# google-research/big_vision

Hardware: NVIDIA H100
Metric: siglip_vit_b16_pairs_per_sec (higher is better)
Workload: dtype bf16

## Files before the change

### big_vision_b200/csrc/gemm.cu

```cuda
#include "common.cuh"
#include "gemm_sched.h"
#include "host_utils.h"
#include "kernels.h"

#include <atomic>

#include <stdlib.h>
#include <string.h>

namespace bv {

namespace {

constexpr int BM = 128;
constexpr int BK = 64;
constexpr int A_STAGE_BYTES = BM * BK * 2;
constexpr int NUM_THREADS = 384;
constexpr int SUB_BYTES = 64 * 64 * 2;

enum : int { EF_BIAS = 0, EF_GELU = 1, EF_RESID = 2, EF_DGELU = 3 };
enum : int { OM_F32 = 0, OM_BF16_ADD = 1, OM_BF16_TMA = 2 };

template <int BN, int OM, int EF>
struct Cfg {
  static constexpr int B_STAGE_BYTES = BN * BK * 2;
  static constexpr int STAGE_BYTES = A_STAGE_BYTES + B_STAGE_BYTES;
  static constexpr int OUTS = OM != OM_BF16_TMA ? 0 : (EF == EF_GELU ? 2 : 1);
  static constexpr int BUF_BYTES = OUTS * SUB_BYTES;
  static constexpr int STAGING_BYTES = 2 * 2 * BUF_BYTES;
  static constexpr int SMEM_LIMIT = 232448 - 2048;
  static constexpr int STAGES_FIT = (SMEM_LIMIT - STAGING_BYTES) / STAGE_BYTES;
  static constexpr int STAGES = STAGES_FIT > 8 ? 8 : STAGES_FIT;
  static constexpr int STAGING_OFFSET = STAGES * STAGE_BYTES;
  static constexpr int BAR_OFFSET = STAGING_OFFSET + STAGING_BYTES;
  static constexpr int SMEM_BYTES = BAR_OFFSET + 256 + 1024;
  static_assert(STAGES >= 3, "shared-memory budget leaves fewer than 3 stages");
};

struct GemmDev {
  GemmSched s;
  int M, N;
  int a_mn, b_mn;
  int reduce_out;
  float alpha;
  const float* bias;
  const bf16* aux;
  void* d; void* d2;
  long long ldd, ldd2, ldaux;
  float* colsum;
  int aux_row_mod;
};

template <int BN, int STAGES, int STAGE_BYTES, int TA, int TB>
__device__ __forceinline__ void mainloop(float (&acc)[BN / 2], uint32_t base, uint32_t bar_base, int cw,
                                         PipeState& ps, int kb0, int kb1) {
  constexpr uint32_t a_lbo = TA ? 8192u : 16u, b_lbo = TB ? 8192u : 16u;
  constexpr uint32_t a_kstep = TA ? 2048u : 32u, b_kstep = TB ? 2048u : 32u;
  int prev_stage = -1;
  for (int kb = kb0; kb < kb1; ++kb) {
    mbar_wait(bar_base + 8u * ps.stage, ps.phase);
    const uint32_t a_s = base + ps.stage * STAGE_BYTES + cw * 8192;
    const uint32_t b_s = base + ps.stage * STAGE_BYTES + A_STAGE_BYTES;
    const uint64_t adesc = wgmma_desc_sw128(a_s, a_lbo, 1024u), bdesc = wgmma_desc_sw128(b_s, b_lbo, 1024u);
    wgmma_fence_regs(acc);
    wgmma_fence();
#pragma unroll
    for (int k = 0; k < BK / 16; ++k) {
      const uint64_t a = adesc + k * (a_kstep >> 4), b = bdesc + k * (b_kstep >> 4);
      const int accumulate = (kb > kb0 || k > 0) ? 1 : 0;
      if constexpr (BN == 256) wgmma_ss_n256<TA, TB>(acc, a, b, accumulate);
      else wgmma_ss_n128<TA, TB>(acc, a, b, accumulate);
    }
    wgmma_commit();
    wgmma_fence_regs(acc);
    wgmma_wait<1>();
    if (prev_stage >= 0 && (threadIdx.x & 127) == 0) mbar_arrive(bar_base + 8u * (STAGES + prev_stage));
    prev_stage = ps.stage;
    ps.advance(STAGES);
  }
  wgmma_wait<0>();
  wgmma_fence_regs(acc);
  if (prev_stage >= 0 && (threadIdx.x & 127) == 0) mbar_arrive(bar_base + 8u * (STAGES + prev_stage));
}

template <bool OUT_F32, int EF>
__device__ __forceinline__ void epi_math(const GemmDev& p, float alpha, float c0, float c1, float b0, float b1,
                                         int row, int col, bool pair, float& v0, float& v1, float& pre0,
                                         float& pre1) {
  constexpr bool HAS_AUX = (EF == EF_RESID || EF == EF_DGELU);
  v0 = c0 * alpha + b0;
  v1 = c1 * alpha + b1;
  float a0 = 0.f, a1 = 0.f;
  if (HAS_AUX) {
    const long long ar = p.aux_row_mod > 0 ? (row % p.aux_row_mod) : row;
    const bf16* ap = p.aux + ar * p.ldaux + col;
    if (pair) {
      const uint32_t q = *reinterpret_cast<const uint32_t*>(ap);
      a0 = bf16_lo(q); a1 = bf16_hi(q);
    } else {
      a0 = __bfloat162float(*ap);
    }
  }
  pre0 = pre1 = 0.f;
  if (EF == EF_GELU) {
    pre0 = round_bf16(v0); pre1 = round_bf16(v1);
    v0 = gelu_tanh_fast(pre0); v1 = gelu_tanh_fast(pre1);
  } else if (EF == EF_RESID) {
    v0 = (OUT_F32 ? v0 : round_bf16(v0)) + a0;
    v1 = (OUT_F32 ? v1 : round_bf16(v1)) + a1;
  } else if (EF == EF_DGELU) {
    v0 *= gelu_tanh_grad_fast(a0);
    v1 *= gelu_tanh_grad_fast(a1);
  }
}


__device__ __forceinline__ void colsum_add(float* colsum, int N, float s0, float s1, int col, int lane) {
  s0 += __shfl_xor_sync(0xffffffffu, s0, 4);
  s0 += __shfl_xor_sync(0xffffffffu, s0, 8);
  s0 += __shfl_xor_sync(0xffffffffu, s0, 16);
  s1 += __shfl_xor_sync(0xffffffffu, s1, 4);
  s1 += __shfl_xor_sync(0xffffffffu, s1, 8);
  s1 += __shfl_xor_sync(0xffffffffu, s1, 16);
  if (lane < 4) {
    if (col < N) atomicAdd(colsum + col, s0);
    if (col + 1 < N) atomicAdd(colsum + col + 1, s1);
  }
}

template <int BN, bool OUT_F32, int EF>
__device__ __forceinline__ void epilogue_regs(const GemmDev& p, const float (&acc)[BN / 2], int m0, int n0,
                                              int cw) {
  const int lane = threadIdx.x & 31, warp = (threadIdx.x >> 5) & 3;
  const int row0 = m0 + cw * 64 + warp * 16 + (lane >> 2);
  const int pM = p.M, pN = p.N;
  const float alpha = p.alpha;
  const bool reduce = p.reduce_out != 0;
#pragma unroll
  for (int j = 0; j < BN / 8; ++j) {
    const int col = n0 + 8 * j + 2 * (lane & 3);
    if (col >= pN) continue;
    const bool pair = col + 1 < pN;
    float b0 = 0.f, b1 = 0.f;
    if (p.bias != nullptr) {
      b0 = __ldg(p.bias + col);
      if (pair) b1 = __ldg(p.bias + col + 1);
    }
#pragma unroll
    for (int h = 0; h < 2; ++h) {
      const int row = row0 + 8 * h;
      if (row >= pM) continue;
      float v0, v1, pre0, pre1;
      epi_math<OUT_F32, EF>(p, alpha, acc[4 * j + 2 * h], acc[4 * j + 2 * h + 1], b0, b1, row, col, pair, v0, v1,
                            pre0, pre1);
      if (OUT_F32) {
        float* dp = static_cast<float*>(p.d) + row * p.ldd + col;
        if (reduce) {
          atomicAdd(dp, v0);
          if (pair) atomicAdd(dp + 1, v1);
        } else if (pair) {
          *reinterpret_cast<float2*>(dp) = make_float2(v0, v1);
        } else {
          *dp = v0;
        }
      } else {
        bf16* dp = static_cast<bf16*>(p.d) + row * p.ldd + col;
        const __nv_bfloat162 o = __floats2bfloat162_rn(v0, v1);
        if (pair) atomicAdd(reinterpret_cast<__nv_bfloat162*>(dp), o);
        else atomicAdd(dp, o.x);
      }
    }
  }
}

template <int BN, int EF, int BUF_BYTES>
__device__ __forceinline__ void epilogue_tma(const GemmDev& p, const CUtensorMap* tmD, const CUtensorMap* tmD2,
                                             const float (&acc)[BN / 2], int m0, int n0, int cw, uint32_t staging,
                                             uint32_t& nstore) {
  const int lane = threadIdx.x & 31, warp = (threadIdx.x >> 5) & 3;
  const bool leader = (threadIdx.x & 127) == 0;
  const int rl0 = warp * 16 + (lane >> 2);
  const int row0 = m0 + cw * 64 + rl0;
  const int pM = p.M, pN = p.N;
  const float alpha = p.alpha;
#pragma unroll
  for (int c = 0; c < BN / 64; ++c) {
    const uint32_t buf = staging + (nstore & 1u) * BUF_BYTES;
    if (leader) tma_store_wait_read<1>();
    named_bar_sync(1 + cw, 128);
    float cs[8][2];
#pragma unroll
    for (int jj = 0; jj < 8; ++jj) {
      const int j = 8 * c + jj;
      const int col = n0 + 8 * j + 2 * (lane & 3);
      cs[jj][0] = cs[jj][1] = 0.f;
      const bool cin = col < pN, pair = col + 1 < pN;
      float b0 = 0.f, b1 = 0.f;
      if (cin && p.bias != nullptr) {
        b0 = __ldg(p.bias + col);
        if (pair) b1 = __ldg(p.bias + col + 1);
      }
#pragma unroll
      for (int h = 0; h < 2; ++h) {
        const int rl = rl0 + 8 * h, row = row0 + 8 * h;
        float v0 = 0.f, v1 = 0.f, pre0 = 0.f, pre1 = 0.f;
        const bool in = cin && row < pM;
        if (in)
          epi_math<false, EF>(p, alpha, acc[4 * j + 2 * h], acc[4 * j + 2 * h + 1], b0, b1, row, col, pair, v0, v1,
                              pre0, pre1);
        const __nv_bfloat162 o = __floats2bfloat162_rn(v0, v1);
        if (in) {
          cs[jj][0] += __low2float(o);
          cs[jj][1] += pair ? __high2float(o) : 0.f;
        }
        const uint32_t off = rl * 128 + ((jj ^ (rl & 7)) << 4) + (lane & 3) * 4;
        asm volatile("st.shared.b32 [%0], %1;" ::"r"(buf + off), "r"(*reinterpret_cast<const uint32_t*>(&o))
                     : "memory");
        if (EF == EF_GELU) {
          const __nv_bfloat162 q = __floats2bfloat162_rn(pre0, pre1);
          asm volatile("st.shared.b32 [%0], %1;" ::"r"(buf + SUB_BYTES + off),
                       "r"(*reinterpret_cast<const uint32_t*>(&q))
                       : "memory");
        }
      }
    }
    fence_proxy_async();
    named_bar_sync(1 + cw, 128);
    if (leader) {
      if (n0 + 64 * c < pN && m0 + cw * 64 < pM) {
        tma_store_2d(tmD, buf, n0 + 64 * c, m0 + cw * 64);
        if (EF == EF_GELU) tma_store_2d(tmD2, buf + SUB_BYTES, n0 + 64 * c, m0 + cw * 64);
      }
      tma_store_commit();
    }
    ++nstore;
    if (p.colsum != nullptr) {
#pragma unroll
      for (int jj = 0; jj < 8; ++jj)
        colsum_add(p.colsum, pN, cs[jj][0], cs[jj][1], n0 + 8 * (8 * c + jj) + 2 * (lane & 3), lane);
    }
  }
}

template <int BN, int OM, int EF>
__global__ void __launch_bounds__(NUM_THREADS, 1)
gemm_kernel(const __grid_constant__ CUtensorMap tmA, const __grid_constant__ CUtensorMap tmB,
            const __grid_constant__ CUtensorMap tmD, const __grid_constant__ CUtensorMap tmD2, const GemmDev p) {
  using C = Cfg<BN, OM, EF>;
  extern __shared__ uint8_t smem_raw[];
  const uint32_t raw_addr = smem_u32(smem_raw);
  const uint32_t base = (raw_addr + 1023u) & ~1023u;
  const uint32_t bar_base = base + C::BAR_OFFSET;
  auto full_bar = [&](int s) { return bar_base + 8u * s; };
  auto empty_bar = [&](int s) { return bar_base + 8u * (C::STAGES + s); };

  const int wg = __shfl_sync(0xffffffffu, static_cast<int>(threadIdx.x >> 7), 0);
  const int units = p.s.units;

  if (threadIdx.x == 0) {
    tma_prefetch_desc(&tmA);
    tma_prefetch_desc(&tmB);
    for (int s = 0; s < C::STAGES; ++s) {
      mbar_init(full_bar(s), 1);
      mbar_init(empty_bar(s), 2);
    }
    fence_barrier_init();
  }
  __syncthreads();

  if (wg == 0) {
    asm volatile("setmaxnreg.dec.sync.aligned.u32 40;");
    if (threadIdx.x == 0) {
      PipeState ps;
      for (int u = blockIdx.x; u < units; u += gridDim.x) {
        const WorkUnit w = gemm_work_unit(p.s, u, BM, BN);
        for (int kb = w.kb0; kb < w.kb1; ++kb) {
          mbar_wait(empty_bar(ps.stage), ps.phase ^ 1u);
          const uint32_t a_s = base + ps.stage * C::STAGE_BYTES;
          const uint32_t b_s = a_s + A_STAGE_BYTES;
          const uint32_t fb = full_bar(ps.stage);
          mbar_expect_tx(fb, C::STAGE_BYTES);
          const int k0 = kb * BK;
          if (p.a_mn) {
#pragma unroll
            for (int j = 0; j < BM / 64; ++j) tma_load_2d(a_s + j * 8192, &tmA, fb, w.m0 + 64 * j, k0);
          } else {
            tma_load_2d(a_s, &tmA, fb, k0, w.m0);
          }
          if (p.b_mn) {
#pragma unroll
            for (int j = 0; j < BN / 64; ++j) tma_load_2d(b_s + j * 8192, &tmB, fb, w.n0 + 64 * j, k0);
          } else {
            tma_load_2d(b_s, &tmB, fb, k0, w.n0);
          }
          ps.advance(C::STAGES);
        }
      }
    }
    return;
  }

  asm volatile("setmaxnreg.inc.sync.aligned.u32 232;");
  const int cw = wg - 1;
  const uint32_t staging = base + C::STAGING_OFFSET + cw * 2 * C::BUF_BYTES;
  uint32_t nstore = 0;
  PipeState ps;
  constexpr int S = C::STAGES, SB = C::STAGE_BYTES;
  for (int u = blockIdx.x; u < units; u += gridDim.x) {
    const WorkUnit w = gemm_work_unit(p.s, u, BM, BN);
    float acc[BN / 2];
    if (p.a_mn) {
      if (p.b_mn) mainloop<BN, S, SB, 1, 1>(acc, base, bar_base, cw, ps, w.kb0, w.kb1);
      else mainloop<BN, S, SB, 1, 0>(acc, base, bar_base, cw, ps, w.kb0, w.kb1);
    } else {
      if (p.b_mn) mainloop<BN, S, SB, 0, 1>(acc, base, bar_base, cw, ps, w.kb0, w.kb1);
      else mainloop<BN, S, SB, 0, 0>(acc, base, bar_base, cw, ps, w.kb0, w.kb1);
    }

    if constexpr (OM == OM_BF16_TMA) epilogue_tma<BN, EF, C::BUF_BYTES>(p, &tmD, &tmD2, acc, w.m0, w.n0, cw, staging, nstore);
    else epilogue_regs<BN, OM == OM_F32, EF>(p, acc, w.m0, w.n0, cw);
  }
  if (OM == OM_BF16_TMA && (threadIdx.x & 127) == 0) tma_store_wait<0>();
}

template <int BN, int OM, int EF>
int launch_cfg(const GemmArgs& g, cudaStream_t stream) {
  using C = Cfg<BN, OM, EF>;
  CUtensorMap tmA, tmB, tmD, tmD2;
  int rc;
  const CUtensorMapDataType bf = CU_TENSOR_MAP_DATA_TYPE_BFLOAT16;
  if (g.a_mn) rc = make_tmap_2d(&tmA, bf, g.A, g.M, g.K, g.lda * 2, 64, 64);
  else        rc = make_tmap_2d(&tmA, bf, g.A, g.K, g.M, g.lda * 2, 64, BM);
  if (rc) return rc;
  if (g.b_mn) rc = make_tmap_2d(&tmB, bf, g.B, g.N, g.K, g.ldb * 2, 64, 64);
  else        rc = make_tmap_2d(&tmB, bf, g.B, g.K, g.N, g.ldb * 2, 64, BN);
  if (rc) return rc;

  GemmDev p;
  const long long tiles = ((g.M + BM - 1) / BM) * ((g.N + BN - 1) / BN);
  if (tiles * ((g.K + BK - 1) / BK) > 0x7fffffffLL) { set_error("bv_gemm: problem too large"); return BV_ERR_INVALID; }
  if (!gemm_make_sched(g.M, g.N, g.K, BM, BN, BK, g.splits, g.reduce_out != 0, num_sms(), &p.s)) {
    set_error("bv_gemm: split-K requires reduce_out=1");
    return BV_ERR_INVALID;
  }
  p.M = (int)g.M; p.N = (int)g.N;
  p.a_mn = g.a_mn; p.b_mn = g.b_mn; p.reduce_out = g.reduce_out;
  p.alpha = g.alpha;
  p.bias = g.bias;
  p.colsum = g.colsum;
  p.aux = reinterpret_cast<const bf16*>(g.aux);
  p.ldaux = g.ldaux;
  p.aux_row_mod = g.aux_row_mod;
  p.d = g.D; p.d2 = g.D2;
  p.ldd = g.ldd; p.ldd2 = g.ldd2;
  memset(&tmD, 0, sizeof(tmD));
  memset(&tmD2, 0, sizeof(tmD2));
  if (OM == OM_BF16_TMA) {
    rc = make_tmap_2d(&tmD, bf, g.D, g.N, g.M, g.ldd * 2, 64, 64);
    if (rc) return rc;
    if (EF == EF_GELU) {
      rc = make_tmap_2d(&tmD2, bf, g.D2, g.N, g.M, g.ldd2 * 2, 64, 64);
      if (rc) return rc;
    }
  }

  auto kern = gemm_kernel<BN, OM, EF>;
  static std::atomic<bool> attr_set[64];
  int dev = 0;
  if (cudaGetDevice(&dev) != cudaSuccess || dev < 0 || dev >= 64) dev = -1;
  if (dev < 0 || !attr_set[dev].load(std::memory_order_acquire)) {
    rc = check_cuda(cudaFuncSetAttribute(kern, cudaFuncAttributeMaxDynamicSharedMemorySize, C::SMEM_BYTES),
                    "cudaFuncSetAttribute(gemm)");
    if (rc) return rc;
    if (dev >= 0) attr_set[dev].store(true, std::memory_order_release);
  }
  const int grid = p.s.units < num_sms() ? p.s.units : num_sms();
  kern<<<grid, NUM_THREADS, C::SMEM_BYTES, stream>>>(tmA, tmB, tmD, tmD2, p);
  return check_cuda(cudaGetLastError(), "gemm_kernel launch");
}

template <int BN>
int dispatch_epi(const GemmArgs& g, cudaStream_t s) {
  const bool f32 = (g.out_dtype == DT_F32), add = !f32 && g.reduce_out;
  switch (g.epi) {
    case EPI_NONE:
    case EPI_BIAS:
      return f32 ? launch_cfg<BN, OM_F32, EF_BIAS>(g, s)
                 : add ? launch_cfg<128, OM_BF16_ADD, EF_BIAS>(g, s) : launch_cfg<BN, OM_BF16_TMA, EF_BIAS>(g, s);
    case EPI_BIAS_RESID:
      return f32 ? launch_cfg<BN, OM_F32, EF_RESID>(g, s)
                 : add ? launch_cfg<128, OM_BF16_ADD, EF_RESID>(g, s) : launch_cfg<BN, OM_BF16_TMA, EF_RESID>(g, s);
    case EPI_BIAS_GELU:
      return launch_cfg<BN, OM_BF16_TMA, EF_GELU>(g, s);
    case EPI_DGELU:
      if (f32) { set_error("bv_gemm: DGELU epilogue writes bf16"); return BV_ERR_INVALID; }
      if (g.aux_row_mod > 0) { set_error("bv_gemm: DGELU takes a row-aligned aux"); return BV_ERR_INVALID; }
      return add ? launch_cfg<128, OM_BF16_ADD, EF_DGELU>(g, s) : launch_cfg<BN, OM_BF16_TMA, EF_DGELU>(g, s);
  }
  set_error("bv_gemm: bad epilogue %d", g.epi);
  return BV_ERR_INVALID;
}

}

int launch_gemm(const GemmArgs& g, cudaStream_t stream) {
  if (g.M <= 0 || g.N <= 0 || g.K <= 0) { set_error("bv_gemm: empty problem"); return BV_ERR_INVALID; }
  if (g.out_dtype == DT_BF16 && ((reinterpret_cast<uintptr_t>(g.D) & 15) || (g.ldd % 8))) {
    set_error("bv_gemm: bf16 output must be 16B aligned with ldd %% 8 == 0"); return BV_ERR_INVALID;
  }
  if (g.out_dtype == DT_F32 && ((reinterpret_cast<uintptr_t>(g.D) & 7) || (g.ldd % 2))) {
    set_error("bv_gemm: fp32 output must be 8B aligned with an even ldd"); return BV_ERR_INVALID;
  }
  if (g.M > 0x7fffffffLL || g.N > 0x7fffffffLL || g.K > 0x7fffffffLL) {
    set_error("bv_gemm: dimension exceeds int32"); return BV_ERR_INVALID;
  }
  if (g.epi < EPI_NONE || g.epi > EPI_DGELU) { set_error("bv_gemm: bad epilogue %d", g.epi); return BV_ERR_INVALID; }
  if ((g.epi == EPI_BIAS_RESID || g.epi == EPI_DGELU) && g.aux == nullptr) {
    set_error("bv_gemm: epilogue %d needs aux", g.epi); return BV_ERR_INVALID;
  }
  if (g.aux != nullptr && ((reinterpret_cast<uintptr_t>(g.aux) & 15) || (g.ldaux % 8))) {
    set_error("bv_gemm: aux must be 16B aligned with ldaux %% 8 == 0"); return BV_ERR_INVALID;
  }
  if (g.bias != nullptr && (reinterpret_cast<uintptr_t>(g.bias) & 15)) {
    set_error("bv_gemm: bias must be 16B aligned"); return BV_ERR_INVALID;
  }
  if (g.epi == EPI_BIAS_GELU && (g.out_dtype != DT_BF16 || g.D2 == nullptr || g.reduce_out)) {
    set_error("bv_gemm: BIAS_GELU needs bf16 output, D2 and no reduce"); return BV_ERR_INVALID;
  }
  if (g.epi == EPI_BIAS_GELU && ((reinterpret_cast<uintptr_t>(g.D2) & 15) || (g.ldd2 % 8))) {
    set_error("bv_gemm: D2 must be 16B aligned with ldd2 %% 8 == 0"); return BV_ERR_INVALID;
  }
  if (g.out_dtype != DT_F32 && g.out_dtype != DT_BF16) { set_error("bv_gemm: bad out dtype"); return BV_ERR_INVALID; }
  if (g.colsum != nullptr && (g.out_dtype != DT_BF16 || g.reduce_out)) {
    set_error("bv_gemm: colsum needs a plain bf16 output"); return BV_ERR_INVALID;
  }
  int bn = g.block_n;
  if (bn == 0) bn = (g.N > 128) ? 256 : 128;
  if (bn == 256) return dispatch_epi<256>(g, stream);
  if (bn == 128) return dispatch_epi<128>(g, stream);
  set_error("bv_gemm: block_n must be 0, 128 or 256");
  return BV_ERR_INVALID;
}

}
```

Baseline: 1856.

## Prefetch residual/dgelu aux tile via TMA into staging during mainloop

For bf16 TMA-store epilogues with a residual or GELU-gradient aux input, the consumer leader issues TMA loads of the aux tile into the output staging buffers after the first k-block's wgmma is issued. The epilogue then reads aux from shared memory instead of doing scattered 4-byte global loads. This overlaps the aux fetch with the matmul. In exchange it enlarges staging (one buffer per 64-column chunk, which can cut pipeline stages for BN=256), drops double-buffered store overlap, and adds a wait for all prior TMA stores before each tile. A separate row-mod residual variant keeps the global-load path.

```diff
diff --git a/big_vision_b200/csrc/gemm.cu b/big_vision_b200/csrc/gemm.cu
--- a/big_vision_b200/csrc/gemm.cu
+++ b/big_vision_b200/csrc/gemm.cu
@@ -18,23 +18,27 @@
 constexpr int NUM_THREADS = 384;
 constexpr int SUB_BYTES = 64 * 64 * 2;
 
-enum : int { EF_BIAS = 0, EF_GELU = 1, EF_RESID = 2, EF_DGELU = 3 };
+enum : int { EF_BIAS = 0, EF_GELU = 1, EF_RESID = 2, EF_DGELU = 3, EF_RESID_ROWMOD = 4 };
 enum : int { OM_F32 = 0, OM_BF16_ADD = 1, OM_BF16_TMA = 2 };
 
 template <int BN, int OM, int EF>
 struct Cfg {
   static constexpr int B_STAGE_BYTES = BN * BK * 2;
   static constexpr int STAGE_BYTES = A_STAGE_BYTES + B_STAGE_BYTES;
+  static constexpr bool AUX_TMA = OM == OM_BF16_TMA && (EF == EF_RESID || EF == EF_DGELU);
   static constexpr int OUTS = OM != OM_BF16_TMA ? 0 : (EF == EF_GELU ? 2 : 1);
   static constexpr int BUF_BYTES = OUTS * SUB_BYTES;
-  static constexpr int STAGING_BYTES = 2 * 2 * BUF_BYTES;
+  static constexpr int BUFS = AUX_TMA ? BN / 64 : 2;
+  static constexpr int STAGING_BYTES = 2 * BUFS * BUF_BYTES;
   static constexpr int SMEM_LIMIT = 232448 - 2048;
   static constexpr int STAGES_FIT = (SMEM_LIMIT - STAGING_BYTES) / STAGE_BYTES;
   static constexpr int STAGES = STAGES_FIT > 8 ? 8 : STAGES_FIT;
   static constexpr int STAGING_OFFSET = STAGES * STAGE_BYTES;
   static constexpr int BAR_OFFSET = STAGING_OFFSET + STAGING_BYTES;
+  static constexpr int AUX_BAR = 2 * STAGES;
   static constexpr int SMEM_BYTES = BAR_OFFSET + 256 + 1024;
   static_assert(STAGES >= 3, "shared-memory budget leaves fewer than 3 stages");
+  static_assert(8 * (AUX_BAR + (AUX_TMA ? 2 * BUFS : 0)) <= 256, "barriers overflow their 256 bytes");
 };
 
 struct GemmDev {
@@ -51,9 +55,9 @@
   int aux_row_mod;
 };
 
-template <int BN, int STAGES, int STAGE_BYTES, int TA, int TB>
+template <int BN, int STAGES, int STAGE_BYTES, int TA, int TB, typename F>
 __device__ __forceinline__ void mainloop(float (&acc)[BN / 2], uint32_t base, uint32_t bar_base, int cw,
-                                         PipeState& ps, int kb0, int kb1) {
+                                         PipeState& ps, int kb0, int kb1, F&& after_first) {
   constexpr uint32_t a_lbo = TA ? 8192u : 16u, b_lbo = TB ? 8192u : 16u;
   constexpr uint32_t a_kstep = TA ? 2048u : 32u, b_kstep = TB ? 2048u : 32u;
   int prev_stage = -1;
@@ -73,6 +77,7 @@
     }
     wgmma_commit();
     wgmma_fence_regs(acc);
+    if (kb == kb0) after_first();
     wgmma_wait<1>();
     if (prev_stage >= 0 && (threadIdx.x & 127) == 0) mbar_arrive(bar_base + 8u * (STAGES + prev_stage));
     prev_stage = ps.stage;
@@ -83,29 +88,28 @@
   if (prev_stage >= 0 && (threadIdx.x & 127) == 0) mbar_arrive(bar_base + 8u * (STAGES + prev_stage));
 }
 
+__device__ __forceinline__ void aux_global(const GemmDev& p, int row, int col, bool pair, float& a0, float& a1) {
+  const long long ar = p.aux_row_mod > 0 ? (row % p.aux_row_mod) : row;
+  const bf16* ap = p.aux + ar * p.ldaux + col;
+  if (pair) {
+    const uint32_t q = *reinterpret_cast<const uint32_t*>(ap);
+    a0 = bf16_lo(q); a1 = bf16_hi(q);
+  } else {
+    a0 = __bfloat162float(*ap);
+    a1 = 0.f;
+  }
+}
+
 template <bool OUT_F32, int EF>
-__device__ __forceinline__ void epi_math(const GemmDev& p, float alpha, float c0, float c1, float b0, float b1,
-                                         int row, int col, bool pair, float& v0, float& v1, float& pre0,
-                                         float& pre1) {
-  constexpr bool HAS_AUX = (EF == EF_RESID || EF == EF_DGELU);
+__device__ __forceinline__ void epi_math(float alpha, float c0, float c1, float b0, float b1, float a0, float a1,
+                                         float& v0, float& v1, float& pre0, float& pre1) {
   v0 = c0 * alpha + b0;
   v1 = c1 * alpha + b1;
-  float a0 = 0.f, a1 = 0.f;
-  if (HAS_AUX) {
-    const long long ar = p.aux_row_mod > 0 ? (row % p.aux_row_mod) : row;
-    const bf16* ap = p.aux + ar * p.ldaux + col;
-    if (pair) {
-      const uint32_t q = *reinterpret_cast<const uint32_t*>(ap);
-      a0 = bf16_lo(q); a1 = bf16_hi(q);
-    } else {
-      a0 = __bfloat162float(*ap);
-    }
-  }
   pre0 = pre1 = 0.f;
   if (EF == EF_GELU) {
     pre0 = round_bf16(v0); pre1 = round_bf16(v1);
     v0 = gelu_tanh_fast(pre0); v1 = gelu_tanh_fast(pre1);
-  } else if (EF == EF_RESID) {
+  } else if (EF == EF_RESID || EF == EF_RESID_ROWMOD) {
     v0 = (OUT_F32 ? v0 : round_bf16(v0)) + a0;
     v1 = (OUT_F32 ? v1 : round_bf16(v1)) + a1;
   } else if (EF == EF_DGELU) {
@@ -150,9 +154,9 @@
     for (int h = 0; h < 2; ++h) {
       const int row = row0 + 8 * h;
       if (row >= pM) continue;
-      float v0, v1, pre0, pre1;
-      epi_math<OUT_F32, EF>(p, alpha, acc[4 * j + 2 * h], acc[4 * j + 2 * h + 1], b0, b1, row, col, pair, v0, v1,
-                            pre0, pre1);
+      float v0, v1, pre0, pre1, a0 = 0.f, a1 = 0.f;
+      if (EF == EF_RESID || EF == EF_DGELU) aux_global(p, row, col, pair, a0, a1);
+      epi_math<OUT_F32, EF>(alpha, acc[4 * j + 2 * h], acc[4 * j + 2 * h + 1], b0, b1, a0, a1, v0, v1, pre0, pre1);
       if (OUT_F32) {
         float* dp = static_cast<float*>(p.d) + row * p.ldd + col;
         if (reduce) {
@@ -176,7 +180,8 @@
 template <int BN, int EF, int BUF_BYTES>
 __device__ __forceinline__ void epilogue_tma(const GemmDev& p, const CUtensorMap* tmD, const CUtensorMap* tmD2,
                                              const float (&acc)[BN / 2], int m0, int n0, int cw, uint32_t staging,
-                                             uint32_t& nstore) {
+                                             uint32_t& nstore, uint32_t aux_bar, uint32_t aux_parity) {
+  constexpr bool AUX_TMA = (EF == EF_RESID || EF == EF_DGELU);
   const int lane = threadIdx.x & 31, warp = (threadIdx.x >> 5) & 3;
   const bool leader = (threadIdx.x & 127) == 0;
   const int rl0 = warp * 16 + (lane >> 2);
@@ -185,9 +190,15 @@
   const float alpha = p.alpha;
 #pragma unroll
   for (int c = 0; c < BN / 64; ++c) {
-    const uint32_t buf = staging + (nstore & 1u) * BUF_BYTES;
-    if (leader) tma_store_wait_read<1>();
-    named_bar_sync(1 + cw, 128);
+    uint32_t buf;
+    if constexpr (AUX_TMA) {
+      buf = staging + c * BUF_BYTES;
+      mbar_wait(aux_bar + 8u * c, aux_parity);
+    } else {
+      buf = staging + (nstore & 1u) * BUF_BYTES;
+      if (leader) tma_store_wait_read<1>();
+      named_bar_sync(1 + cw, 128);
+    }
     float cs[8][2];
 #pragma unroll
     for (int jj = 0; jj < 8; ++jj) {
@@ -203,17 +214,25 @@
 #pragma unroll
       for (int h = 0; h < 2; ++h) {
         const int rl = rl0 + 8 * h, row = row0 + 8 * h;
+        const uint32_t off = rl * 128 + ((jj ^ (rl & 7)) << 4) + (lane & 3) * 4;
         float v0 = 0.f, v1 = 0.f, pre0 = 0.f, pre1 = 0.f;
         const bool in = cin && row < pM;
-        if (in)
-          epi_math<false, EF>(p, alpha, acc[4 * j + 2 * h], acc[4 * j + 2 * h + 1], b0, b1, row, col, pair, v0, v1,
-                              pre0, pre1);
+        if (in) {
+          float a0 = 0.f, a1 = 0.f;
+          if constexpr (AUX_TMA) {
+            uint32_t q;
+            asm volatile("ld.shared.b32 %0, [%1];" : "=r"(q) : "r"(buf + off));
+            a0 = bf16_lo(q); a1 = bf16_hi(q);
+          } else if constexpr (EF == EF_RESID_ROWMOD) {
+            aux_global(p, row, col, pair, a0, a1);
+          }
+          epi_math<false, EF>(alpha, acc[4 * j + 2 * h], acc[4 * j + 2 * h + 1], b0, b1, a0, a1, v0, v1, pre0, pre1);
+        }
         const __nv_bfloat162 o = __floats2bfloat162_rn(v0, v1);
         if (in) {
           cs[jj][0] += __low2float(o);
           cs[jj][1] += pair ? __high2float(o) : 0.f;
         }
-        const uint32_t off = rl * 128 + ((jj ^ (rl & 7)) << 4) + (lane & 3) * 4;
         asm volatile("st.shared.b32 [%0], %1;" ::"r"(buf + off), "r"(*reinterpret_cast<const uint32_t*>(&o))
                      : "memory");
         if (EF == EF_GELU) {
@@ -233,11 +252,27 @@
       }
       tma_store_commit();
     }
-    ++nstore;
+    if (!AUX_TMA) ++nstore;
     if (p.colsum != nullptr) {
 #pragma unroll
       for (int jj = 0; jj < 8; ++jj)
         colsum_add(p.colsum, pN, cs[jj][0], cs[jj][1], n0 + 8 * (8 * c + jj) + 2 * (lane & 3), lane);
+    }
+  }
+}
+
+template <int BN>
+__device__ __forceinline__ void issue_aux_loads(const CUtensorMap* tmAux, int M, int N, int m0, int n0, int cw,
+                                                uint32_t staging, uint32_t aux_bar) {
+  tma_store_wait_read<0>();
+#pragma unroll
+  for (int c = 0; c < BN / 64; ++c) {
+    const uint32_t bar = aux_bar + 8u * c;
+    if (n0 + 64 * c < N && m0 + cw * 64 < M) {
+      mbar_expect_tx(bar, SUB_BYTES);
+      tma_load_2d(staging + c * SUB_BYTES, tmAux, bar, n0 + 64 * c, m0 + cw * 64);
+    } else {
+      mbar_arrive(bar);
     }
   }
 }
@@ -245,7 +280,8 @@
 template <int BN, int OM, int EF>
 __global__ void __launch_bounds__(NUM_THREADS, 1)
 gemm_kernel(const __grid_constant__ CUtensorMap tmA, const __grid_constant__ CUtensorMap tmB,
-            const __grid_constant__ CUtensorMap tmD, const __grid_constant__ CUtensorMap tmD2, const GemmDev p) {
+            const __grid_constant__ CUtensorMap tmD, const __grid_constant__ CUtensorMap tmD2,
+            const __grid_constant__ CUtensorMap tmAux, const GemmDev p) {
   using C = Cfg<BN, OM, EF>;
   extern __shared__ uint8_t smem_raw[];
   const uint32_t raw_addr = smem_u32(smem_raw);
@@ -260,9 +296,13 @@
   if (threadIdx.x == 0) {
     tma_prefetch_desc(&tmA);
     tma_prefetch_desc(&tmB);
+    if (C::AUX_TMA) tma_prefetch_desc(&tmAux);
     for (int s = 0; s < C::STAGES; ++s) {
       mbar_init(full_bar(s), 1);
       mbar_init(empty_bar(s), 2);
+    }
+    if (C::AUX_TMA) {
+      for (int b = 0; b < 2 * C::BUFS; ++b) mbar_init(bar_base + 8u * (C::AUX_BAR + b), 1);
     }
     fence_barrier_init();
   }
@@ -302,22 +342,30 @@
 
   asm volatile("setmaxnreg.inc.sync.aligned.u32 232;");
   const int cw = wg - 1;
-  const uint32_t staging = base + C::STAGING_OFFSET + cw * 2 * C::BUF_BYTES;
-  uint32_t nstore = 0;
+  const uint32_t staging = base + C::STAGING_OFFSET + cw * C::BUFS * C::BUF_BYTES;
+  const uint32_t aux_bar = bar_base + 8u * (C::AUX_BAR + cw * C::BUFS);
+  const bool leader = (threadIdx.x & 127) == 0;
+  uint32_t nstore = 0, nunit = 0;
   PipeState ps;
   constexpr int S = C::STAGES, SB = C::STAGE_BYTES;
-  for (int u = blockIdx.x; u < units; u += gridDim.x) {
+  for (int u = blockIdx.x; u < units; u += gridDim.x, ++nunit) {
     const WorkUnit w = gemm_work_unit(p.s, u, BM, BN);
+    auto after_first = [&]() {
+      if constexpr (C::AUX_TMA) {
+        if (leader) issue_aux_loads<BN>(&tmAux, p.M, p.N, w.m0, w.n0, cw, staging, aux_bar);
+      }
+    };
     float acc[BN / 2];
     if (p.a_mn) {
-      if (p.b_mn) mainloop<BN, S, SB, 1, 1>(acc, base, bar_base, cw, ps, w.kb0, w.kb1);
-      else mainloop<BN, S, SB, 1, 0>(acc, base, bar_base, cw, ps, w.kb0, w.kb1);
+      if (p.b_mn) mainloop<BN, S, SB, 1, 1>(acc, base, bar_base, cw, ps, w.kb0, w.kb1, after_first);
+      else mainloop<BN, S, SB, 1, 0>(acc, base, bar_base, cw, ps, w.kb0, w.kb1, after_first);
     } else {
-      if (p.b_mn) mainloop<BN, S, SB, 0, 1>(acc, base, bar_base, cw, ps, w.kb0, w.kb1);
-      else mainloop<BN, S, SB, 0, 0>(acc, base, bar_base, cw, ps, w.kb0, w.kb1);
-    }
-
-    if constexpr (OM == OM_BF16_TMA) epilogue_tma<BN, EF, C::BUF_BYTES>(p, &tmD, &tmD2, acc, w.m0, w.n0, cw, staging, nstore);
+      if (p.b_mn) mainloop<BN, S, SB, 0, 1>(acc, base, bar_base, cw, ps, w.kb0, w.kb1, after_first);
+      else mainloop<BN, S, SB, 0, 0>(acc, base, bar_base, cw, ps, w.kb0, w.kb1, after_first);
+    }
+
+    if constexpr (OM == OM_BF16_TMA)
+      epilogue_tma<BN, EF, C::BUF_BYTES>(p, &tmD, &tmD2, acc, w.m0, w.n0, cw, staging, nstore, aux_bar, nunit & 1u);
     else epilogue_regs<BN, OM == OM_F32, EF>(p, acc, w.m0, w.n0, cw);
   }
   if (OM == OM_BF16_TMA && (threadIdx.x & 127) == 0) tma_store_wait<0>();
@@ -326,7 +374,7 @@
 template <int BN, int OM, int EF>
 int launch_cfg(const GemmArgs& g, cudaStream_t stream) {
   using C = Cfg<BN, OM, EF>;
-  CUtensorMap tmA, tmB, tmD, tmD2;
+  CUtensorMap tmA, tmB, tmD, tmD2, tmAux;
   int rc;
   const CUtensorMapDataType bf = CU_TENSOR_MAP_DATA_TYPE_BFLOAT16;
   if (g.a_mn) rc = make_tmap_2d(&tmA, bf, g.A, g.M, g.K, g.lda * 2, 64, 64);
@@ -355,6 +403,7 @@
   p.ldd = g.ldd; p.ldd2 = g.ldd2;
   memset(&tmD, 0, sizeof(tmD));
   memset(&tmD2, 0, sizeof(tmD2));
+  memset(&tmAux, 0, sizeof(tmAux));
   if (OM == OM_BF16_TMA) {
     rc = make_tmap_2d(&tmD, bf, g.D, g.N, g.M, g.ldd * 2, 64, 64);
     if (rc) return rc;
@@ -362,6 +411,10 @@
       rc = make_tmap_2d(&tmD2, bf, g.D2, g.N, g.M, g.ldd2 * 2, 64, 64);
       if (rc) return rc;
     }
+  }
+  if (C::AUX_TMA) {
+    rc = make_tmap_2d(&tmAux, bf, g.aux, g.N, g.M, g.ldaux * 2, 64, 64);
+    if (rc) return rc;
   }
 
   auto kern = gemm_kernel<BN, OM, EF>;
@@ -375,7 +428,7 @@
     if (dev >= 0) attr_set[dev].store(true, std::memory_order_release);
   }
   const int grid = p.s.units < num_sms() ? p.s.units : num_sms();
-  kern<<<grid, NUM_THREADS, C::SMEM_BYTES, stream>>>(tmA, tmB, tmD, tmD2, p);
+  kern<<<grid, NUM_THREADS, C::SMEM_BYTES, stream>>>(tmA, tmB, tmD, tmD2, tmAux, p);
   return check_cuda(cudaGetLastError(), "gemm_kernel launch");
 }
 
@@ -388,8 +441,10 @@
       return f32 ? launch_cfg<BN, OM_F32, EF_BIAS>(g, s)
                  : add ? launch_cfg<128, OM_BF16_ADD, EF_BIAS>(g, s) : launch_cfg<BN, OM_BF16_TMA, EF_BIAS>(g, s);
     case EPI_BIAS_RESID:
-      return f32 ? launch_cfg<BN, OM_F32, EF_RESID>(g, s)
-                 : add ? launch_cfg<128, OM_BF16_ADD, EF_RESID>(g, s) : launch_cfg<BN, OM_BF16_TMA, EF_RESID>(g, s);
+      if (f32) return launch_cfg<BN, OM_F32, EF_RESID>(g, s);
+      if (add) return launch_cfg<128, OM_BF16_ADD, EF_RESID>(g, s);
+      return g.aux_row_mod > 0 ? launch_cfg<BN, OM_BF16_TMA, EF_RESID_ROWMOD>(g, s)
+                               : launch_cfg<BN, OM_BF16_TMA, EF_RESID>(g, s);
     case EPI_BIAS_GELU:
       return launch_cfg<BN, OM_BF16_TMA, EF_GELU>(g, s);
     case EPI_DGELU:
```

Measured after the change: 2063, median of 6. 1.11x the previous value.
